# Greketrotny/RayZath

Hardware: AMD Instinct MI355X
Metric: Mrays/s (path segments, primary+secondary) at 1920x1080 depth 8 (higher is better)
Workload: dtype f32; 1 GPU; Cornell box 1920x1080 depth 8; max_depth=8, triangles=16, instances=8, traversal=workgroup-binned, integrator=CPU kernel (parity-checked), pipeline=resident (one kernel per step)

## Files before the change

### rayzath_amd/csrc/hiprz_device.hpp

```cpp
#pragma once
#include <hip/hip_runtime.h>
#include <stdint.h>

#include "hiprz.h"
#include "hiprz_end.hpp"
#include "hiprz_lds.hpp"
#include "hiprz_shard.hpp"

#define RZ_DEV __device__ __forceinline__
#include "hiprz_flat_pick.hpp"
#include "hiprz_pair_pick.hpp"

namespace hiprz {

#ifndef RZ_FUSED_SHARED_RCP
#define RZ_FUSED_SHARED_RCP 0
#endif
#ifndef RZ_TRACE_SHARED_RCP
#define RZ_TRACE_SHARED_RCP 1
#endif
#ifndef RZ_BATCH_SHARED_RCP
#define RZ_BATCH_SHARED_RCP 1
#endif
#ifndef RZ_FLAT_PACKED_BOXES
// ... 65 lines not shown
    uint32_t world_advance;
    uint32_t walk_h;
    uint32_t off_pairs;
    const float4* nodes64;
    uint32_t shadow_variant;
    const float4* shadow_nodes64;
    const uint32_t* shadow_order;
    uint32_t shadow_root;
    uint32_t sort_variant;
};

RZ_DEV void repoint_hot(DScene& v, const unsigned char* base) {
    v.nodes = reinterpret_cast<const float4*>(base + v.off_nodes);
    v.tlas_order = reinterpret_cast<const uint32_t*>(base + v.off_tlas_order);
    v.instances = reinterpret_cast<const float4*>(base + v.off_instances);
    v.tris = reinterpret_cast<const float4*>(base + v.off_tris);
    v.tri_attrs = reinterpret_cast<const float4*>(base + v.off_tri_attrs);
    v.materials = reinterpret_cast<const float4*>(base + v.off_materials);
    v.inst_materials = reinterpret_cast<const int32_t*>(base + v.off_inst_materials);
}

static_assert(sizeof(DScene) == 256, "off_pairs fills a padding word: the kernels' argument layout is what it was");
RZ_DEV const unsigned char* pair_section(const DScene& s) { return reinterpret_cast<const unsigned char*>(s.nodes) - s.off_nodes + s.off_pairs; }

struct DCamera {
    float position[3];
    float x_axis[3], y_axis[3], z_axis[3];
    uint32_t width, height;
    float tan_half_fov, aspect_ratio;
    float near_, far_;
    float focal_distance, aperture, exposure_time;
};

struct DConfig {
    uint32_t max_depth, spot_samples, direct_samples, seed;
    uint32_t flags;
};

struct DFrame {
    float4* st0;
    float4* st1;
    float2* st2;
    float4* accum;
    float4* hit0;
    uint32_t* hit1;
    float* depth;
// ... 1944 lines not shown
RZ_DEV col4 fetch_rgba8(const DScene& s, int32_t tex, float u, float v, Counters& cnt) {
    return from_u8(*reinterpret_cast<const uint32_t*>(s.texels + texel_offset<COUNT>(s, tex, u, v, 4u, cnt)));
}
template <bool COUNT>
RZ_DEV float fetch_r8(const DScene& s, int32_t tex, float u, float v, Counters& cnt) {
    return float(s.texels[texel_offset<COUNT>(s, tex, u, v, 1u, cnt)]) / 255.0f;
}
template <bool COUNT>
RZ_DEV float fetch_r32f(const DScene& s, int32_t tex, float u, float v, Counters& cnt) {
    return *reinterpret_cast<const float*>(s.texels + texel_offset<COUNT>(s, tex, u, v, 4u, cnt));
}

struct Surface {
    uint32_t surface_material, behind_material;
    float u, v;
    v3 normal, mapped_normal;
    col4 color;
    float metalness, roughness, emission;
    float fresnel, reflectance, tint_factor;
    float refr_x, refr_y;
    float surface_scattering;
};

template <bool COUNT, bool TEX = true>
RZ_DEV void analyze_intersection(const DScene& s, const Hit& hit, Surface& sf, Material& m, Counters& cnt, bool compat_filtering = false) {
    const uint32_t inst = uint32_t(hit.instance);
    const float4 i1 = s.instances[7 * inst + 1], i2 = s.instances[7 * inst + 2],
                 i3 = s.instances[7 * inst + 3], i4 = s.instances[7 * inst + 4];
    const v3 scale = xyz(i1), xa = xyz(i2), ya = xyz(i3), za = xyz(i4);
    const uint32_t material_base = __float_as_uint(i1.w), material_count = __float_as_uint(i2.w);

    const float4 ta = s.tris[3 * hit.triangle];
    const uint32_t flags = __float_as_uint(ta.w);
    const float4* at = s.tri_attrs + 6 * size_t(hit.triangle);

    uint32_t slot = flags & HIPRZ_TRI_MATERIAL_MASK;
    if (slot > 63u) slot = 63u;
    int32_t mat = -1;
    if (slot < material_count) mat = s.inst_materials[material_base + slot];
    sf.surface_material = mat < 0 ? HIPRZ_MATERIAL_DEFAULT : uint32_t(mat);
    sf.behind_material = hit.external ? sf.surface_material : HIPRZ_MATERIAL_WORLD;
    m = load_material(s, sf.surface_material);

    const bool has_texcrds = (flags & HIPRZ_TRI_HAS_TEXCRDS) != 0;
    float4 uv12 = make_float4(0, 0, 0, 0), uv3 = make_float4(0, 0, 0, 0);
    if (has_texcrds) {
        uv12 = at[4], uv3 = at[5];
        const float b3 = 1.0f - hit.bx - hit.by;
// ... 437 lines not shown
```

### rayzath_amd/csrc/hiprz_end.hpp

```cpp
#pragma once
#define RZ_END 0xFFFFFFFFu
#define RZ_PAIR_RECORD_BYTES 72u
```

### rayzath_amd/csrc/hiprz_kernels.hpp

```cpp
#pragma once
#include <hip/hip_runtime.h>

#include "hiprz.h"
#include "hiprz_device.hpp"
#include "hiprz_compat.hpp"

namespace hiprz {

struct PathState {
    Ray ray;
    col4 color;
    uint32_t material, depth;
};

template <bool LDS_SCENE>
RZ_DEV uint32_t stage_scene(DScene& s, unsigned char* lds) {
    if constexpr (LDS_SCENE) {
        float4* dst = reinterpret_cast<float4*>(lds);
        const uint32_t n16 = s.hot_bytes >> 4;
        for (uint32_t i = threadIdx.x; i < n16; i += 256u) dst[i] = s.hot[i];
        __syncthreads();
        repoint_hot(s, lds);
        return s.hot_bytes;
    }
// ... 61 lines not shown
        return closest_hit_flat<COUNT, RCP>(s, world, workspace, active, ray, hit, cnt);
    } else if constexpr (MODE == 2) {
        return closest_hit_binned<COUNT, RCP>(s, workspace, active, ray, hit, cnt);
    } else {
        hit.instance = -1, hit.triangle = 0, hit.bx = hit.by = 0.0f, hit.external = true;
        return active ? closest_hit<MODE, COUNT, RCP>(s, lds_column, ray, hit, cnt) : 0;
    }
}

template <bool COUNT, bool TEX, bool COMPAT>
RZ_DEV void fetch_color_emission(const DScene& s, const Material& m, uint32_t flags, bool filtering, Surface& sf, Counters& cnt) {
    if (COMPAT && (flags & HIPRZ_COMPAT_TEXTURE_MULT)) {
        sf.color = compat_opacity_color<COUNT>(s, m, sf.u, sf.v, true, filtering, cnt);
        sf.emission = m.emission;
        if (m.emission_map >= 0) sf.emission *= filtering ? compat_fetch<COUNT>(s, m.emission_map, sf.u, sf.v, cnt).r : fetch_r32f<COUNT>(s, m.emission_map, sf.u, sf.v, cnt);
    } else {
        sf.color = from_u8(m.color);
        if (TEX && m.texture >= 0) sf.color = filtering ? compat_fetch<COUNT>(s, m.texture, sf.u, sf.v, cnt) : fetch_rgba8<COUNT>(s, m.texture, sf.u, sf.v, cnt);
        sf.color.a = 1.0f - sf.color.a;
        sf.emission = TEX && m.emission_map >= 0 ? (filtering ? compat_fetch<COUNT>(s, m.emission_map, sf.u, sf.v, cnt).r : fetch_r32f<COUNT>(s, m.emission_map, sf.u, sf.v, cnt)) : m.emission;
    }
}

template <bool COUNT, int SHADOW = 1>
RZ_DEV void shade_segment(const DScene& s, const DCamera& cam, const DConfig& cfg, const PixelId& p, PathState& ps, uint32_t pass,
                          int found, const Hit& hit, const ShadowCtx& lds_column, Counters& cnt, col4& final_color, bool& path_continues,
                          Rng* shared_rng = nullptr) {
    constexpr bool COMPAT = shadow_mode_compat(SHADOW);
    Ray& ray = ps.ray;
    col4& ray_color = ps.color;
    uint32_t& ray_material = ps.material;
    uint32_t& depth = ps.depth;
    const uint32_t pixel_idx = p.y * cam.width + p.x;
    Rng own_rng(float(p.x) / float(cam.width), float(p.y) / float(cam.height), seed_value(cfg.seed, pass, (pixel_idx + depth) & 255u));
    Rng& rng = COMPAT ? *shared_rng : own_rng;
    const bool filtering = COMPAT && (cfg.flags & HIPRZ_COMPAT_FILTERING) != 0u;

    final_color = splat(0.0f);
    Surface sf;
    sf.surface_material = sf.behind_material = HIPRZ_MATERIAL_WORLD;
    sf.u = sf.v = 0.0f;
    sf.normal = sf.mapped_normal = V3(0.0f, 0.0f, 0.0f);
    sf.fresnel = 1.0f, sf.reflectance = 0.0f, sf.tint_factor = 0.0f, sf.refr_x = sf.refr_y = 0.0f;
    sf.metalness = sf.roughness = 0.0f;

    constexpr bool TEX = SHADOW != RZ_SHADOW_PLAIN;
    Material m;
    if (found == 2) {
        analyze_intersection<COUNT, TEX>(s, hit, sf, m, cnt, filtering);
    } else if (COMPAT && found == 3) {
        m = load_material(s, ray_material);
        sf.surface_material = sf.behind_material = ray_material;
        sf.normal = sf.mapped_normal = ray.d;
        if (TEX) {
            sf.u = -(0.5f + (RZ_ATAN2F(ray.d.z, ray.d.x) / (RZ_PI_F * 2.0f)));
            sf.v = 0.5f + (RZ_ASINF(ray.d.y) / RZ_PI_F);
        }
    } else {
        m = load_material(s, HIPRZ_MATERIAL_WORLD);
        if (TEX && (found == 1 || (COMPAT && found == 0))) {
            sf.u = -(0.5f + (RZ_ATAN2F(ray.d.z, ray.d.x) / (RZ_PI_F * 2.0f)));
            sf.v = 0.5f + (RZ_ASINF(ray.d.y) / RZ_PI_F);
        }
    }
    sf.surface_scattering = m.scattering;
    fetch_color_emission<COUNT, TEX, COMPAT>(s, m, cfg.flags, filtering, sf, cnt);
    if (COMPAT && (cfg.flags & HIPRZ_COMPAT_BEER_LAMBERT)) {
        col4 medium = from_u8(load_material(s, ray_material).color);
        medium.a = 1.0f - medium.a;
        ray_color = ray_color * (medium * RZ_POWF(medium.a, ray.far_));
    }
    if (sf.emission > 0.0f) final_color = final_color + (ray_color * sf.color) * sf.emission;
// ... 17 lines not shown
        if constexpr (shadow_mode_defers(SHADOW)) {
            lds_column.defer_done = true;
            lds_column.defer_a = ray_color, lds_column.defer_b = lerp(splat(1.0f), sf.color, sf.metalness);
        } else if constexpr (SHADOW == RZ_SHADOW_NONE || SHADOW == RZ_SHADOW_PLAIN) {
            (void)direct;
        } else {
            final_color = final_color + (direct * ray_color) * lerp(splat(1.0f), sf.color, sf.metalness);
        }
        ray_color = lerp(ray_color, ray_color * sf.color, sf.tint_factor);
    }
    path_continues = depth < cfg.max_depth;
    if (path_continues) {
        ray.o = point;
        ray.d = next_direction;
    } else {
        RZ_COUNT(finished);
        generate_antialiased_ray(cam, ray, p.x, p.y, rng);
        ray_material = HIPRZ_MATERIAL_WORLD;
        ray_color = splat(1.0f);
        depth = 0u;
    }
}

template <bool FIRST, bool COUNT, int SHADOW = 1>
RZ_DEV void shade_and_store(const DScene& s, const DCamera& cam, const DConfig& cfg, const DFrame& f, const PixelId& p, PathState& ps,
                            int found, const Hit& hit, const ShadowCtx& lds_column, Counters& cnt, Rng* shared_rng = nullptr) {
    const float hit_distance = ps.ray.far_;
    col4 final_color;
    bool path_continues;
    shade_segment<COUNT, SHADOW>(s, cam, cfg, p, ps, FIRST ? 0u : *f.pass, found, hit, lds_column, cnt, final_color, path_continues, shared_rng);
    const Ray& ray = ps.ray;
    const col4& ray_color = ps.color;
    const uint32_t ray_material = ps.material, depth = ps.depth;

    if constexpr (FIRST) f.depth[p.local] = hit_distance;
    if constexpr (shadow_mode_defers(SHADOW)) {
        const uint32_t bits = (path_continues ? 1u : 0u) | (lds_column.defer_done ? 2u : 0u) | (lds_column.defer_mask << 2);
        float4* rec = f.nee + size_t(p.local) * f.nee_quads;
        rec[0] = make_float4(final_color.r, final_color.g, final_color.b, __uint_as_float(bits));
        if (lds_column.defer_done) {
            rec[2] = make_float4(lds_column.defer_a.r, lds_column.defer_a.g, lds_column.defer_a.b, lds_column.defer_a.a);
            rec[3] = make_float4(lds_column.defer_b.r, lds_column.defer_b.g, lds_column.defer_b.b, lds_column.defer_b.a);
        }
    } else {
        col4 value;
        if constexpr (FIRST) {
            value = col4{final_color.r, final_color.g, final_color.b, float(!path_continues)};
        } else {
            const float4 acc = f.accum[p.local];
            value = col4{acc.x + final_color.r, acc.y + final_color.g, acc.z + final_color.b, acc.w + float(!path_continues)};
        }
        f.accum[p.local] = make_float4(value.r, value.g, value.b, value.a);
    }
// ... 47 lines not shown
    DScene s = scene_in;
    unsigned char* workspace = rz_lds + stage_scene<LDS_SCENE>(s, rz_lds);
    uint32_t* lds_column = stack_column<MODE>(workspace);
    const PixelId p = pixel_of_thread(f, cam, blockIdx.x, threadIdx.x);
    Counters cnt;
    PathState ps;
    load_path<FIRST>(f, cam, p, ps);
    Hit hit;
    int found;
    const auto world = walk_world<MODE>(s);
    if constexpr (binned_mode(MODE)) {
        static_assert(kFusedParkBytes == 4u * 256u * sizeof(uint32_t), "park [4][256]");
        uint32_t* park = reinterpret_cast<uint32_t*>(workspace + BinnedLds::kFixedBytes + (s.world_stack_entries + s.mesh_stack_entries) * 1024u);
        park[0 * 256 + threadIdx.x] = __float_as_uint(ps.color.r), park[1 * 256 + threadIdx.x] = __float_as_uint(ps.color.g);
        park[2 * 256 + threadIdx.x] = __float_as_uint(ps.color.b), park[3 * 256 + threadIdx.x] = ps.material | (ps.depth << 16);
        found = trace_path<MODE, COUNT, RZ_FUSED_SHARED_RCP != 0>(s, world, workspace, lds_column, p.active, ps.ray, hit, cnt);
        ps.color = col4{__uint_as_float(park[0 * 256 + threadIdx.x]), __uint_as_float(park[1 * 256 + threadIdx.x]),
                        __uint_as_float(park[2 * 256 + threadIdx.x]), 1.0f};
        const uint32_t bits = park[3 * 256 + threadIdx.x];
        ps.material = bits & 0xFFFFu, ps.depth = bits >> 16;
    } else {
        found = trace_path<MODE, COUNT, RZ_FUSED_SHARED_RCP != 0>(s, world, workspace, lds_column, p.active, ps.ray, hit, cnt);
    }
    if (p.active) shade_and_store<FIRST, COUNT>(s, cam, cfg, f, p, ps, found, hit, ShadowCtx{lds_column, TopCache{nullptr, nullptr, 0u}}, cnt);
    flush_counters<COUNT>(f, p.active ? 1u : 0u, cnt);
}

template <bool COUNT, int MODE, int SHADING, bool SC1 = false>
RZ_DEV void batch_tile(const DScene& s, const DCamera& cam, const DConfig& cfg, const DFrame& f, unsigned char* workspace, uint32_t* park,
                       const PixelId& p, uint32_t pass0, uint32_t n_passes, bool tonemap_out, Counters& cnt) {
    uint32_t* lds_column = stack_column<MODE>(workspace);
    PathState ps;
    load_path<false, SC1>(f, cam, p, ps);
    {
        const float4 acc = p.active ? load_state<SC1>(f.accum + p.local) : make_float4(0.0f, 0.0f, 0.0f, 0.0f);
        park[4 * 256] = __float_as_uint(acc.x), park[5 * 256] = __float_as_uint(acc.y);
        park[6 * 256] = __float_as_uint(acc.z), park[7 * 256] = __float_as_uint(acc.w);
    }
    const auto world = walk_world<MODE>(s);
    for (uint32_t i = 0; i < n_passes; ++i) {
        if (i != 0u && p.active) {
            ps.ray.d = normalized(ps.ray.d);
            ps.ray.near_ = 0.0f, ps.ray.far_ = RZ_FLT_MAX;
            if (ps.depth == 0u) ps.ray.near_ = cam.near_, ps.ray.far_ = cam.far_;
        }
        Hit hit;
        int found;
        if constexpr (binned_mode(MODE)) {
            park[0 * 256] = __float_as_uint(ps.color.r), park[1 * 256] = __float_as_uint(ps.color.g);
            park[2 * 256] = __float_as_uint(ps.color.b), park[3 * 256] = ps.material | (ps.depth << 16);
            found = trace_path<MODE, COUNT, RZ_BATCH_SHARED_RCP != 0>(s, world, workspace, lds_column, p.active, ps.ray, hit, cnt);
            ps.color = col4{__uint_as_float(park[0 * 256]), __uint_as_float(park[1 * 256]), __uint_as_float(park[2 * 256]), 1.0f};
            const uint32_t bits = park[3 * 256];
            ps.material = bits & 0xFFFFu, ps.depth = bits >> 16;
        } else {
            found = trace_path<MODE, COUNT, RZ_BATCH_SHARED_RCP != 0>(s, world, workspace, lds_column, p.active, ps.ray, hit, cnt);
        }
        if (p.active) {
            col4 final_color;
            bool path_continues;
            shade_segment<COUNT, SHADING>(s, cam, cfg, p, ps, pass0 + i, found, hit, ShadowCtx{lds_column, TopCache{nullptr, nullptr, 0u}}, cnt, final_color, path_continues);
            park[4 * 256] = __float_as_uint(__uint_as_float(park[4 * 256]) + final_color.r);
            park[5 * 256] = __float_as_uint(__uint_as_float(park[5 * 256]) + final_color.g);
            park[6 * 256] = __float_as_uint(__uint_as_float(park[6 * 256]) + final_color.b);
            park[7 * 256] = __float_as_uint(__uint_as_float(park[7 * 256]) + float(!path_continues));
        }
    }
    if (p.active) {
        const float4 acc = make_float4(__uint_as_float(park[4 * 256]), __uint_as_float(park[5 * 256]), __uint_as_float(park[6 * 256]),
                                       __uint_as_float(park[7 * 256]));
        store_state<SC1>(f.accum + p.local, acc);
        store_state<SC1>(f.st0 + p.local, make_float4(ps.ray.o.x, ps.ray.o.y, ps.ray.o.z, ps.ray.d.x));
        store_state<SC1>(f.st1 + p.local, make_float4(ps.ray.d.y, ps.ray.d.z, ps.color.r, ps.color.g));
        store_state<SC1>(f.st2 + p.local, make_float2(ps.color.b, __uint_as_float((ps.material & 0xFFFFu) | (ps.depth << 16))));
        if (tonemap_out) f.rgba8[p.local] = tonemap(col4{acc.x, acc.y, acc.z, acc.w}, cam.aperture, cam.exposure_time);
    }
}

template <bool COUNT, int MODE, bool LDS_SCENE, int SHADING, int WAVES = RZ_MIN_WAVES>
__global__ void __launch_bounds__(256, WAVES) rz_batch_kernel(const DScene scene_in, const DCamera cam, const DConfig cfg, const DFrame f,
                                                                      uint32_t n_passes, uint32_t park_offset) {
    extern __shared__ __attribute__((aligned(16))) unsigned char rz_lds[];
    const unsigned long long t_start = __builtin_readcyclecounter();
    const uint32_t unit = (f.launch_order && !f.xcd_swizzle) ? f.launch_order[blockIdx.x] : blockIdx.x;
    const PixelId p = pixel_of_thread(f, cam, unit, threadIdx.x);
    if (!p.tile_inside) return;
    DScene s = scene_in;
    unsigned char* workspace = rz_lds + stage_scene<LDS_SCENE>(s, rz_lds);
    Counters cnt;
    uint32_t* park = reinterpret_cast<uint32_t*>(workspace + park_offset) + threadIdx.x;
    batch_tile<COUNT, MODE, SHADING>(s, cam, cfg, f, workspace, park, p, *f.pass, n_passes, true, cnt);
    if (f.unit_cost && threadIdx.x == 0u) {
        const unsigned long long dt = (__builtin_readcyclecounter() - t_start) >> 4;
        f.unit_cost[unit] = dt < 0x00FFFFFFull ? uint32_t(dt) : 0x00FFFFFFu;
    }
    flush_counters<COUNT>(f, p.active ? n_passes : 0u, cnt);
}

template <bool COUNT, int MODE, bool LDS_SCENE, int SHADING, int WAVES = RZ_MIN_WAVES>
__global__ void __launch_bounds__(256, WAVES) rz_batch_seg_kernel(const DScene scene_in, const DCamera cam, const DConfig cfg, const DFrame f,
                                                                          uint32_t n_passes, uint32_t park_offset, uint32_t segments, uint32_t n_units,
                                                                          uint32_t* seg) {
    extern __shared__ __attribute__((aligned(16))) unsigned char rz_lds[];
    DScene s = scene_in;
    unsigned char* workspace = rz_lds + stage_scene<LDS_SCENE>(s, rz_lds);
    uint32_t* park = reinterpret_cast<uint32_t*>(workspace + park_offset) + threadIdx.x;
    uint32_t* item_slot = reinterpret_cast<uint32_t*>(workspace + park_offset + 8u * 1024u);
    const uint32_t n_items = segments * n_units, pass_base = *f.pass;
    uint32_t base = 0u;
    if (threadIdx.x == 0u) base = __hip_atomic_load(&seg[2], __ATOMIC_RELAXED, __HIP_MEMORY_SCOPE_AGENT);
    for (;;) {
        if (threadIdx.x == 0u) item_slot[0] = __hip_atomic_fetch_add(&seg[0], 1u, __ATOMIC_RELAXED, __HIP_MEMORY_SCOPE_AGENT);
        __syncthreads();
        const uint32_t item = item_slot[0];
        if (item >= n_items) break;
        const uint32_t k = item / n_units, j = item - k * n_units;
        const uint32_t unit = (f.launch_order && !f.xcd_swizzle) ? f.launch_order[j] : j;
        const PixelId p = pixel_of_thread(f, cam, unit, threadIdx.x);
        if (p.tile_inside) {
            if (k != 0u) {
                if (threadIdx.x == 0u) {
                    for (uint32_t guard = 0u; __hip_atomic_load(&seg[kSegFlags + unit], __ATOMIC_RELAXED, __HIP_MEMORY_SCOPE_AGENT) != base + k;) {
                        __builtin_amdgcn_s_sleep(2);
                        if (++guard > kSegWaitLimit) break;
                    }
                    __builtin_amdgcn_fence(__ATOMIC_ACQUIRE, "wavefront");
                }
                __syncthreads();
            }
            const unsigned long long t_start = __builtin_readcyclecounter();
            const uint32_t first = k * n_passes / segments, end = (k + 1u) * n_passes / segments;
            Counters cnt;
            batch_tile<COUNT, MODE, SHADING, true>(s, cam, cfg, f, workspace, park, p, pass_base + first, end - first, k + 1u == segments, cnt);
            if (f.unit_cost && threadIdx.x == 0u) {
                const uint32_t before = k != 0u ? __hip_atomic_load(&f.unit_cost[unit], __ATOMIC_RELAXED, __HIP_MEMORY_SCOPE_AGENT) : 0u;
                const unsigned long long dt = ((__builtin_readcyclecounter() - t_start) >> 4) + before;
                __hip_atomic_store(&f.unit_cost[unit], dt < 0x00FFFFFFull ? uint32_t(dt) : 0x00FFFFFFu, __ATOMIC_RELAXED, __HIP_MEMORY_SCOPE_AGENT);
            }
            flush_counters<COUNT>(f, p.active ? end - first : 0u, cnt);
            if (k + 1u != segments) {
                asm volatile("s_waitcnt vmcnt(0)" ::: "memory");
                __syncthreads();
                if (threadIdx.x == 0u) __hip_atomic_store(&seg[kSegFlags + unit], base + k + 1u, __ATOMIC_RELAXED, __HIP_MEMORY_SCOPE_AGENT);
            }
        }
        __syncthreads();
    }
    if (threadIdx.x == 0u && __hip_atomic_fetch_add(&seg[1], 1u, __ATOMIC_ACQ_REL, __HIP_MEMORY_SCOPE_AGENT) == gridDim.x - 1u) {
        __hip_atomic_store(&seg[0], 0u, __ATOMIC_RELAXED, __HIP_MEMORY_SCOPE_AGENT);
        __hip_atomic_store(&seg[1], 0u, __ATOMIC_RELAXED, __HIP_MEMORY_SCOPE_AGENT);
        __hip_atomic_store(&seg[2], base + segments, __ATOMIC_RELAXED, __HIP_MEMORY_SCOPE_AGENT);
    }
}

template <bool COUNT, int SHADING, int MINW, bool ONE_LEAF_WORLD = false>
__global__ void __launch_bounds__(64, MINW) rz_wave_batch_kernel(const DScene s, const DCamera cam, const DConfig cfg, const DFrame f, uint32_t n_passes) {
// ... 161 lines not shown
        for (uint32_t i = threadIdx.x; i < top_n; i += 256u) ls[i] = s.node_skip[i];
        __syncthreads();
        shadow.lds_column = nullptr;
        shadow.top = TopCache{ln, ls, top_n};
    }
    const PixelId p = pixel_of_thread(f, cam, blockIdx.x, threadIdx.x);
    Counters cnt;
    if (p.active) {
        PathState ps;
        load_path<FIRST>(f, cam, p, ps);
        const float4 h0 = f.hit0[p.local];
        const uint32_t h1 = f.hit1[p.local];
        Hit hit;
        const int found = int((h1 >> 29) & 3u);
        ps.ray.far_ = h0.x;
        hit.bx = h0.y, hit.by = h0.z, hit.triangle = __float_as_uint(h0.w);
        hit.instance = found == 2 ? int32_t(h1 & 0x1FFFFFFFu) : -1;
        hit.external = (h1 & 0x80000000u) != 0u;
        shadow.nee = f.nee + size_t(p.local) * f.nee_quads;
        if constexpr (shadow_mode_compat(SHADOW)) {
            const uint32_t pass = FIRST ? 0u : *f.pass, pixel_idx = p.y * cam.width + p.x;
            Rng rng(float(p.x) / float(cam.width), float(p.y) / float(cam.height), seed_value(cfg.seed, pass, (pixel_idx + ps.depth) & 255u));
            if ((cfg.flags & HIPRZ_COMPAT_SCATTERING) && material_scattering(s, ps.material) > 1.0e-4f) (void)rng.unsignedUniform();
            shade_and_store<FIRST, COUNT, SHADOW>(s, cam, cfg, f, p, ps, found, hit, shadow, cnt, &rng);
        } else {
            shade_and_store<FIRST, COUNT, SHADOW>(s, cam, cfg, f, p, ps, found, hit, shadow, cnt);
        }
    } else if (f.sort_key && p.local < f.n_local_tiles * 256u) {
        f.sort_key[p.local] = 0x00FFFFFFu;
        if (f.shadow_key) f.shadow_key[p.local] = 0x00FFFFFFu;
    }
    flush_counters<COUNT>(f, p.active ? 1u : 0u, cnt);
}

template <bool FIRST, bool COUNT, int MINW>
__global__ void __launch_bounds__(64, MINW) rz_shadow_kernel(const DScene s, const DCamera cam, const DConfig cfg, const DFrame f, uint32_t top_n) {
    extern __shared__ __attribute__((aligned(16))) unsigned char rz_lds[];
    float4* ln = reinterpret_cast<float4*>(rz_lds);
    uint32_t* ls = reinterpret_cast<uint32_t*>(rz_lds + top_n * 32u);
    for (uint32_t i = threadIdx.x; i < 2u * top_n; i += 64u) ln[i] = s.nodes[i];
    for (uint32_t i = threadIdx.x; i < top_n; i += 64u) ls[i] = s.node_skip[i];
    const uint32_t slot = blockIdx.x * 64u + threadIdx.x;
    const uint32_t* order = f.shadow_perm ? f.shadow_perm : f.perm;
    const PixelId p = pixel_of_local(f, cam, order ? order[slot] : slot);
    Counters cnt;
    if (p.active) {
        const ShadowCtx sc{nullptr, TopCache{ln, ls, top_n}};
        const float4* rec = f.nee + size_t(p.local) * f.nee_quads;
        const float4 base = rec[0];
// ... 182 lines not shown
```

### rayzath_amd/csrc/hiprz_scene.hip

```cpp
#include <hip/hip_runtime.h>

#include <algorithm>
#include <cstdio>
#include <cstdlib>
#include <cstring>
#include <string>
#include <vector>

#include "hiprz.h"
#include "hiprz_ctx.hpp"
#include "hiprz_device.hpp"
#include "hiprz_scene_host.hpp"

using namespace hiprz;

#define RZ_FANOUT_OTHER_DEVICES(c, call)                                                                                       \
    for (hiprz_ctx* p : (c)->peers) {                                                                                         \
        if (p->device == (c)->device) continue;                                                                               \
        const int rz_rc = (call);                                                                                             \
        if (rz_rc != HIPRZ_OK) return fail(c, rz_rc, "device " + std::to_string(p->device) + ": " + p->error);              \
    }

namespace {

// ... 46 lines not shown
uint32_t env_u32(const char* name, uint32_t otherwise) {
    const char* v = std::getenv(name);
    return v ? uint32_t(std::atoi(v)) : otherwise;
}
uint32_t sort_variant_for(const hiprz_ctx* c, uint32_t n_lights) { return n_lights && c->shadow_sort == 0 ? 0u : 4u; }

int build_shadow_world_tree(hiprz_ctx* c, const std::vector<hiprz_instance>& dinst, DScene& d) {
    d.shadow_nodes64 = nullptr, d.shadow_order = nullptr, d.shadow_root = RZ_END;
    const std::vector<uint32_t>& members = c->world_members;
    if (!c->shadow_tree || members.empty() || members.size() > 160u) return HIPRZ_OK;
    std::vector<uint32_t> rec, order;
    build_shadow_tree(dinst, members, rec, order);
    (void)hipSetDevice(c->device);
    RZ_HIP(c, c->shadow_nodes64.resize(rec.size()));
    RZ_HIP(c, c->shadow_order.resize(order.size()));
    RZ_HIP(c, hipStreamSynchronize(c->stream));
    RZ_HIP(c, hipMemcpy(c->shadow_nodes64.ptr, rec.data(), rec.size() * sizeof(uint32_t), hipMemcpyHostToDevice));
    RZ_HIP(c, hipMemcpy(c->shadow_order.ptr, order.data(), order.size() * sizeof(uint32_t), hipMemcpyHostToDevice));
    d.shadow_nodes64 = reinterpret_cast<const float4*>(c->shadow_nodes64.ptr), d.shadow_order = c->shadow_order.ptr, d.shadow_root = 0u;
    return HIPRZ_OK;
}


int copy_scene(hiprz_ctx* c, const hiprz_scene& sc, const PackedScene& packed, bool device_trees) {
    (void)hipSetDevice(c->device);
    if (packed.pair_section.empty()) {
        RZ_HIP(c, c->hot.assign(packed.blob.data(), packed.blob.size(), c->stream));
    } else {
        std::vector<uint8_t> hot(packed.blob);
        hot.insert(hot.end(), packed.pair_section.begin(), packed.pair_section.end());
        RZ_HIP(c, c->hot.assign(hot.data(), hot.size(), c->stream));
        RZ_HIP(c, hipStreamSynchronize(c->stream));
    }
    RZ_HIP(c, c->node_skip.assign(packed.skip.data(), packed.skip.size(), c->stream));
    if (device_trees) {
        hiprz_node unused{};
        unused.meta = HIPRZ_NODE_LEAF;
        std::vector<hiprz_node> all(packed.node_capacity, unused);
        std::copy(packed.nodes.begin(), packed.nodes.end(), all.begin());
        RZ_HIP(c, c->dev_nodes.assign(reinterpret_cast<const uint8_t*>(all.data()), all.size() * sizeof(hiprz_node), c->stream));
        RZ_HIP(c, hipStreamSynchronize(c->stream));
    }
    RZ_HIP(c, c->nodes64.assign(packed.nodes64.data(), packed.nodes64.size(), c->stream));
    RZ_HIP(c, c->textures.assign(sc.textures, sc.n_textures, c->stream));
    RZ_HIP(c, c->texels.assign(sc.texels, sc.texel_bytes, c->stream));
    RZ_HIP(c, c->spot_lights.assign(sc.spot_lights, sc.n_spot_lights, c->stream));
    RZ_HIP(c, c->direct_lights.assign(sc.direct_lights, sc.n_direct_lights, c->stream));
    RZ_HIP(c, hipStreamSynchronize(c->stream));
    return HIPRZ_OK;
}

void bind_tunables(hiprz_ctx* c, DScene& d, uint32_t n_lights) {
    d.walk_k = env_u32("HIPRZ_WALK_K", 4u), d.walk_l = env_u32("HIPRZ_WALK_L", 8u);
// ... 82 lines not shown
        rc = derive_tables(scene, chk, derived);
    }
    if (message && len) std::snprintf(message, len, "%s", chk.error.c_str());
    return rc;
}

int hiprz_upload_scene(hiprz_ctx* c, const hiprz_scene* sc) {
    if (!c) return HIPRZ_ERR_INVALID;
    RZ_FANOUT_OTHER_DEVICES(c, hiprz_upload_scene(p, sc));
    SceneChange change(c, SceneChange::kInvalidateGraphs | SceneChange::kResolvePeerPipelines);
    StageTimer timer;
    std::string error;
    SceneCheck chk;
    if (check_scene(sc, chk) != HIPRZ_OK) return fail(c, HIPRZ_ERR_INVALID, "upload_scene: " + chk.error);
    c->build_sah = c->device_sah || c->tree_mode == HIPRZ_TREE_AUTO;
    ChosenTrees trees;
    if (choose_trees(sc, c->tree_mode, kLdsSceneLimit, chk, trees, error) != HIPRZ_OK) return fail(c, HIPRZ_ERR_INVALID, error);
    if (trees.own_trees) c->timings.set("rebuild mesh trees", timer.ms());
    DerivedTables derived;
    if (derive_tables(&trees.scene, chk, derived) != HIPRZ_OK) return fail(c, HIPRZ_ERR_INVALID, "upload_scene: " + chk.error);
    c->have_scene = false;
    PackedScene packed;
    if (pack_scene(trees, std::move(derived), packed, error) != HIPRZ_OK) return scene_lost(c, fail(c, HIPRZ_ERR_INVALID, error));
    int rc = copy_scene(c, trees.scene, packed, trees.device_trees());
    if (rc != HIPRZ_OK) return scene_lost(c, rc);
    bind_scene(c, trees, packed, chk);
    if (trees.device_trees()) rc = build_device_trees(c, packed);
    if (rc != HIPRZ_OK) return scene_lost(c, rc);
    rc = build_shadow_world_tree(c, packed.instances, c->dscene);
    if (rc != HIPRZ_OK) return scene_lost(c, rc);
    c->have_scene = true;
    resolve_pipeline(c);
    c->timings.set("upload scene", timer.ms());
    return restart_after_geometry_change(c);
}

int hiprz_update_shading(hiprz_ctx* c, const hiprz_material* materials, uint32_t n_materials, const hiprz_spot_light* spot_lights,
                         uint32_t n_spot_lights, const hiprz_direct_light* direct_lights, uint32_t n_direct_lights) {
    if (!c) return HIPRZ_ERR_INVALID;
    RZ_FANOUT_OTHER_DEVICES(c, hiprz_update_shading(p, materials, n_materials, spot_lights, n_spot_lights, direct_lights, n_direct_lights));
    SceneChange change(c, SceneChange::kInPlace);
    if (!c->have_scene) return fail(c, HIPRZ_ERR_STATE, "update_shading before upload_scene");
    const uint32_t uploaded = (c->dscene.off_inst_materials - c->dscene.off_materials) / uint32_t(sizeof(hiprz_material));
    if (!materials || n_materials < 2u || ((n_materials * sizeof(hiprz_material) + 15u) & ~size_t(15)) != size_t(c->dscene.off_inst_materials - c->dscene.off_materials))
        return fail(c, HIPRZ_ERR_INVALID, "update_shading: the scene was uploaded with " + std::to_string(uploaded) + " material slots");
    if ((n_spot_lights && !spot_lights) || (n_direct_lights && !direct_lights)) return fail(c, HIPRZ_ERR_INVALID, "update_shading: null array with non-zero count");
    std::vector<hiprz_texture> tex(c->n_textures);
// ... 116 lines not shown
```

### rayzath_amd/csrc/hiprz_scene_host.cpp

```cpp
#include "hiprz_scene_host.hpp"

#include <algorithm>

namespace hiprz {

namespace {
struct TreeCheck {
    const hiprz_scene* sc;
    std::vector<uint32_t>& skip;
    std::vector<uint8_t> visited;
    uint32_t max_depth = 0;
    std::string error;
    std::vector<uint32_t> world_leaves;

    bool walk(uint32_t root, bool is_world) {
        struct Item {
            uint32_t node, skip, depth;
        };
        std::vector<Item> stack{{root, RZ_END, 1u}};
        while (!stack.empty()) {
            const Item it = stack.back();
            stack.pop_back();
            if (it.node >= sc->n_nodes) return err("node index out of range");
            if (visited[it.node]) return err("node reachable twice (trees must be disjoint and acyclic)");
            visited[it.node] = 1;
// ... 355 lines not shown
                }
            }
            table[i] = uint16_t(first_of_root[root]), any = true;
        }
        if (any && table_bytes + records.size() <= kPairSectionLimit) {
            out.pair_section.assign((table_bytes + records.size() + 15u) & ~size_t(15), 0);
            std::memcpy(out.pair_section.data(), table.data(), table_bytes);
            if (!records.empty()) std::memcpy(out.pair_section.data() + table_bytes, records.data(), records.size());
        }
        if (out.hot_bytes() > 0xFFFFFFF0ull) {
            error = "scene geometry exceeds 4 GiB";
            return HIPRZ_ERR_INVALID;
        }
    }
    std::vector<uint8_t> member(sc->n_instances ? sc->n_instances : 1u, 0);
    for (uint32_t k = 0; k < sc->n_tlas_order; ++k)
        if (sc->tlas_order[k] < sc->n_instances) member[sc->tlas_order[k]] = 1;
    out.world_members.clear();
    for (uint32_t i = 0; i < sc->n_instances; ++i)
        if (member[i]) out.world_members.push_back(i);
    return HIPRZ_OK;
}

uint32_t enter_device_roots(std::vector<hiprz_instance>& instances, const std::vector<uint32_t>& instance_mesh, const std::vector<DeviceMesh>& meshes,
                            uint32_t world_slots) {
    for (size_t i = 0; i < instances.size(); ++i)
        if (instance_mesh[i] != RZ_END && meshes[instance_mesh[i]].region != RZ_END) instances[i].blas_root = meshes[instance_mesh[i]].region;
    uint32_t emitted = world_slots;
    for (const auto& m : meshes) emitted += m.n_slots;
    return emitted;
}

void build_shadow_tree(const std::vector<hiprz_instance>& dinst, const std::vector<uint32_t>& members, std::vector<uint32_t>& rec,
                       std::vector<uint32_t>& order) {
    auto box_of = [&](uint32_t i) { return packed_instance_box(dinst[i]); };
    auto grow = [](InstanceBox& b, const InstanceBox& o) {
        for (int a = 0; a < 3; ++a) b.mn[a] = std::min(b.mn[a], o.mn[a]), b.mx[a] = std::max(b.mx[a], o.mx[a]);
    };
    auto area = [](const InstanceBox& b) {
        const float x = b.mx[0] - b.mn[0], y = b.mx[1] - b.mn[1], z = b.mx[2] - b.mn[2];
        return x * y + y * z + z * x;
    };
    const uint32_t n = uint32_t(members.size());
    order = members, rec.assign(size_t(2u * n) * 16u, RZ_END);
    std::vector<uint32_t> sorted, best;
    std::vector<float> left_area;
// ... 50 lines not shown
```

### rayzath_amd/csrc/hiprz_scene_host.hpp

```cpp
#pragma once
#include <cstdint>
#include <cstring>
#include <string>
#include <vector>

#include "hiprz.h"
#include "hiprz_end.hpp"

namespace hiprz {

constexpr uint32_t kLeafMax = 4u;
constexpr uint32_t kPairRecordBytes = RZ_PAIR_RECORD_BYTES;
constexpr uint16_t kPairNone = 0xFFFFu;
constexpr size_t kPairSectionLimit = 8u * 0xFFFEu;

struct DeviceMesh {
    uint32_t tri_first = 0, n_tris = 0;
    uint32_t ref_first = 0;
    uint32_t region = 0xFFFFFFFFu;
    uint32_t leaf_slot = 0xFFFFFFFFu;
    uint32_t n_slots = 0;
    float bb_min[3] = {0, 0, 0}, bb_max[3] = {0, 0, 0};
};
uint32_t device_build_regions(std::vector<DeviceMesh>& meshes, uint32_t first_free_slot);
// ... 66 lines not shown
int choose_trees(const hiprz_scene* sc, uint32_t tree_mode, size_t lds_limit, SceneCheck& chk, ChosenTrees& out, std::string& error);

struct PackedScene {
    std::vector<uint8_t> blob;
    uint32_t off_nodes = 0, off_tlas_order = 0, off_instances = 0, off_tris = 0, off_tri_attrs = 0, off_materials = 0, off_inst_materials = 0;
    std::vector<uint32_t> new_index;
    std::vector<hiprz_node> nodes;
    std::vector<uint32_t> skip;
    std::vector<uint32_t> nodes64;
    std::vector<hiprz_instance> instances;
    std::vector<uint32_t> world_members;
    bool fast_div = true;
    float bounds_min[3] = {0, 0, 0}, bounds_scale[3] = {0, 0, 0};
    uint32_t tlas_root = 0;
    bool flat_world = false;
    std::vector<uint8_t> pair_section;
    size_t hot_bytes() const { return blob.size() + pair_section.size(); }
    std::vector<DeviceMesh> device_meshes;
    std::vector<uint32_t> instance_mesh;
    uint32_t world_region = 0, node_capacity = 0;
};
int pack_scene(const ChosenTrees& trees, DerivedTables&& derived, PackedScene& out, std::string& error, bool pair_records = true);

uint32_t enter_device_roots(std::vector<hiprz_instance>& instances, const std::vector<uint32_t>& instance_mesh, const std::vector<DeviceMesh>& meshes,
                            uint32_t world_slots);

void build_shadow_tree(const std::vector<hiprz_instance>& instances, const std::vector<uint32_t>& members, std::vector<uint32_t>& records,
                       std::vector<uint32_t>& order);

}
```

Baseline: 12430 Mrays/s.

## Precompute per-instance-triangle surface normal records in the hot scene section

```diff
diff --git a/rayzath_amd/csrc/hiprz_device.hpp b/rayzath_amd/csrc/hiprz_device.hpp
--- a/rayzath_amd/csrc/hiprz_device.hpp
+++ b/rayzath_amd/csrc/hiprz_device.hpp
@@ -111,6 +111,11 @@
 
 static_assert(sizeof(DScene) == 256, "off_pairs fills a padding word: the kernels' argument layout is what it was");
 RZ_DEV const unsigned char* pair_section(const DScene& s) { return reinterpret_cast<const unsigned char*>(s.nodes) - s.off_nodes + s.off_pairs; }
+
+#ifndef RZ_SURFACE_RECORDS
+#define RZ_SURFACE_RECORDS 1
+#endif
+RZ_DEV const float4* surface_section(const DScene& s) { return s.hot + ((s.hot_bytes + 15u) >> 4); }
 
 struct DCamera {
     float position[3];
@@ -2101,8 +2106,47 @@
     float surface_scattering;
 };
 
-template <bool COUNT, bool TEX = true>
+template <bool TEX>
+RZ_DEV bool surface_from_record(const DScene& s, const Hit& hit, Surface& sf, Material& m) {
+    const float4* section = surface_section(s);
+    const uint32_t pair = reinterpret_cast<const uint32_t*>(section)[uint32_t(hit.instance)] + hit.triangle;
+    const float4* rec = section + ((s.n_instances + 3u) >> 2) + (size_t(pair) * 4u + (hit.external ? 2u : 0u));
+    const float4 ra = rec[0], rb = rec[1];
+    const uint32_t valid = __float_as_uint(rb.w);
+    if (!(valid & RZ_SURFACE_NORMAL_VALID)) return false;
+    sf.surface_material = __float_as_uint(ra.w);
+    sf.behind_material = hit.external ? sf.surface_material : HIPRZ_MATERIAL_WORLD;
+    m = load_material(s, sf.surface_material);
+    if (TEX && m.normal_map >= 0) return false;
+    sf.normal = xyz(ra);
+    if (TEX || !(valid & RZ_SURFACE_MAPPED_VALID)) {
+        const uint32_t flags = __float_as_uint(s.tris[3 * hit.triangle].w);
+        const float4* at = s.tri_attrs + 6 * size_t(hit.triangle);
+        if (TEX && (flags & HIPRZ_TRI_HAS_TEXCRDS)) {
+            const float4 uv12 = at[4], uv3 = at[5];
+            const float b3 = 1.0f - hit.bx - hit.by;
+            sf.u = uv12.x * b3 + uv12.z * hit.bx + uv3.x * hit.by;
+            sf.v = uv12.y * b3 + uv12.w * hit.bx + uv3.y * hit.by;
+        }
+        if (!(valid & RZ_SURFACE_MAPPED_VALID)) {
+            const uint32_t inst = uint32_t(hit.instance);
+            const v3 scale = xyz(s.instances[7 * inst + 1]), xa = xyz(s.instances[7 * inst + 2]), ya = xyz(s.instances[7 * inst + 3]),
+                     za = xyz(s.instances[7 * inst + 4]);
+            v3 mn = xyz(at[3]);
+            if (flags & HIPRZ_TRI_HAS_NORMALS) mn = normalized(xyz(at[0]) * (1.0f - hit.bx - hit.by) + xyz(at[1]) * hit.bx + xyz(at[2]) * hit.by);
+            sf.mapped_normal = normalized(transform_forward(xa, ya, za, mn / scale)) * (float(hit.external) * 2.0f - 1.0f);
+            return true;
+        }
+    }
+    sf.mapped_normal = xyz(rb);
+    return true;
+}
+
+template <bool COUNT, bool TEX = true, bool RECORDS = false>
 RZ_DEV void analyze_intersection(const DScene& s, const Hit& hit, Surface& sf, Material& m, Counters& cnt, bool compat_filtering = false) {
+    if constexpr (RECORDS) {
+        if (surface_from_record<TEX>(s, hit, sf, m)) return;
+    }
     const uint32_t inst = uint32_t(hit.instance);
     const float4 i1 = s.instances[7 * inst + 1], i2 = s.instances[7 * inst + 2],
                  i3 = s.instances[7 * inst + 3], i4 = s.instances[7 * inst + 4];
diff --git a/rayzath_amd/csrc/hiprz_end.hpp b/rayzath_amd/csrc/hiprz_end.hpp
--- a/rayzath_amd/csrc/hiprz_end.hpp
+++ b/rayzath_amd/csrc/hiprz_end.hpp
@@ -1,3 +1,6 @@
 #pragma once
 #define RZ_END 0xFFFFFFFFu
 #define RZ_PAIR_RECORD_BYTES 72u
+#define RZ_SURFACE_RECORD_BYTES 32u
+#define RZ_SURFACE_NORMAL_VALID 1u
+#define RZ_SURFACE_MAPPED_VALID 2u
diff --git a/rayzath_amd/csrc/hiprz_kernels.hpp b/rayzath_amd/csrc/hiprz_kernels.hpp
--- a/rayzath_amd/csrc/hiprz_kernels.hpp
+++ b/rayzath_amd/csrc/hiprz_kernels.hpp
@@ -107,7 +107,8 @@
     }
 }
 
-template <bool COUNT, int SHADOW = 1>
+constexpr bool surface_records(bool lds_scene) { return lds_scene && RZ_SURFACE_RECORDS != 0; }
+template <bool COUNT, int SHADOW = 1, bool RECORDS = false>
 RZ_DEV void shade_segment(const DScene& s, const DCamera& cam, const DConfig& cfg, const PixelId& p, PathState& ps, uint32_t pass,
                           int found, const Hit& hit, const ShadowCtx& lds_column, Counters& cnt, col4& final_color, bool& path_continues,
                           Rng* shared_rng = nullptr) {
@@ -132,7 +133,7 @@
     constexpr bool TEX = SHADOW != RZ_SHADOW_PLAIN;
     Material m;
     if (found == 2) {
-        analyze_intersection<COUNT, TEX>(s, hit, sf, m, cnt, filtering);
+        analyze_intersection<COUNT, TEX, RECORDS>(s, hit, sf, m, cnt, filtering);
     } else if (COMPAT && found == 3) {
         m = load_material(s, ray_material);
         sf.surface_material = sf.behind_material = ray_material;
@@ -196,13 +197,13 @@
     }
 }
 
-template <bool FIRST, bool COUNT, int SHADOW = 1>
+template <bool FIRST, bool COUNT, int SHADOW = 1, bool RECORDS = false>
 RZ_DEV void shade_and_store(const DScene& s, const DCamera& cam, const DConfig& cfg, const DFrame& f, const PixelId& p, PathState& ps,
                             int found, const Hit& hit, const ShadowCtx& lds_column, Counters& cnt, Rng* shared_rng = nullptr) {
     const float hit_distance = ps.ray.far_;
     col4 final_color;
     bool path_continues;
-    shade_segment<COUNT, SHADOW>(s, cam, cfg, p, ps, FIRST ? 0u : *f.pass, found, hit, lds_column, cnt, final_color, path_continues, shared_rng);
+    shade_segment<COUNT, SHADOW, RECORDS>(s, cam, cfg, p, ps, FIRST ? 0u : *f.pass, found, hit, lds_column, cnt, final_color, path_continues, shared_rng);
     const Ray& ray = ps.ray;
     const col4& ray_color = ps.color;
     const uint32_t ray_material = ps.material, depth = ps.depth;
@@ -296,11 +297,11 @@
     } else {
         found = trace_path<MODE, COUNT, RZ_FUSED_SHARED_RCP != 0>(s, world, workspace, lds_column, p.active, ps.ray, hit, cnt);
     }
-    if (p.active) shade_and_store<FIRST, COUNT>(s, cam, cfg, f, p, ps, found, hit, ShadowCtx{lds_column, TopCache{nullptr, nullptr, 0u}}, cnt);
+    if (p.active) shade_and_store<FIRST, COUNT, 1, surface_records(LDS_SCENE)>(s, cam, cfg, f, p, ps, found, hit, ShadowCtx{lds_column, TopCache{nullptr, nullptr, 0u}}, cnt);
     flush_counters<COUNT>(f, p.active ? 1u : 0u, cnt);
 }
 
-template <bool COUNT, int MODE, int SHADING, bool SC1 = false>
+template <bool COUNT, int MODE, int SHADING, bool SC1 = false, bool RECORDS = false>
 RZ_DEV void batch_tile(const DScene& s, const DCamera& cam, const DConfig& cfg, const DFrame& f, unsigned char* workspace, uint32_t* park,
                        const PixelId& p, uint32_t pass0, uint32_t n_passes, bool tonemap_out, Counters& cnt) {
     uint32_t* lds_column = stack_column<MODE>(workspace);
@@ -333,7 +334,7 @@
         if (p.active) {
             col4 final_color;
             bool path_continues;
-            shade_segment<COUNT, SHADING>(s, cam, cfg, p, ps, pass0 + i, found, hit, ShadowCtx{lds_column, TopCache{nullptr, nullptr, 0u}}, cnt, final_color, path_continues);
+            shade_segment<COUNT, SHADING, RECORDS>(s, cam, cfg, p, ps, pass0 + i, found, hit, ShadowCtx{lds_column, TopCache{nullptr, nullptr, 0u}}, cnt, final_color, path_continues);
             park[4 * 256] = __float_as_uint(__uint_as_float(park[4 * 256]) + final_color.r);
             park[5 * 256] = __float_as_uint(__uint_as_float(park[5 * 256]) + final_color.g);
             park[6 * 256] = __float_as_uint(__uint_as_float(park[6 * 256]) + final_color.b);
@@ -363,7 +364,7 @@
     unsigned char* workspace = rz_lds + stage_scene<LDS_SCENE>(s, rz_lds);
     Counters cnt;
     uint32_t* park = reinterpret_cast<uint32_t*>(workspace + park_offset) + threadIdx.x;
-    batch_tile<COUNT, MODE, SHADING>(s, cam, cfg, f, workspace, park, p, *f.pass, n_passes, true, cnt);
+    batch_tile<COUNT, MODE, SHADING, false, surface_records(LDS_SCENE)>(s, cam, cfg, f, workspace, park, p, *f.pass, n_passes, true, cnt);
     if (f.unit_cost && threadIdx.x == 0u) {
         const unsigned long long dt = (__builtin_readcyclecounter() - t_start) >> 4;
         f.unit_cost[unit] = dt < 0x00FFFFFFull ? uint32_t(dt) : 0x00FFFFFFu;
@@ -405,7 +406,7 @@
             const unsigned long long t_start = __builtin_readcyclecounter();
             const uint32_t first = k * n_passes / segments, end = (k + 1u) * n_passes / segments;
             Counters cnt;
-            batch_tile<COUNT, MODE, SHADING, true>(s, cam, cfg, f, workspace, park, p, pass_base + first, end - first, k + 1u == segments, cnt);
+            batch_tile<COUNT, MODE, SHADING, true, surface_records(LDS_SCENE)>(s, cam, cfg, f, workspace, park, p, pass_base + first, end - first, k + 1u == segments, cnt);
             if (f.unit_cost && threadIdx.x == 0u) {
                 const uint32_t before = k != 0u ? __hip_atomic_load(&f.unit_cost[unit], __ATOMIC_RELAXED, __HIP_MEMORY_SCOPE_AGENT) : 0u;
                 const unsigned long long dt = ((__builtin_readcyclecounter() - t_start) >> 4) + before;
@@ -613,9 +614,9 @@
             const uint32_t pass = FIRST ? 0u : *f.pass, pixel_idx = p.y * cam.width + p.x;
             Rng rng(float(p.x) / float(cam.width), float(p.y) / float(cam.height), seed_value(cfg.seed, pass, (pixel_idx + ps.depth) & 255u));
             if ((cfg.flags & HIPRZ_COMPAT_SCATTERING) && material_scattering(s, ps.material) > 1.0e-4f) (void)rng.unsignedUniform();
-            shade_and_store<FIRST, COUNT, SHADOW>(s, cam, cfg, f, p, ps, found, hit, shadow, cnt, &rng);
+            shade_and_store<FIRST, COUNT, SHADOW, surface_records(LDS_SCENE)>(s, cam, cfg, f, p, ps, found, hit, shadow, cnt, &rng);
         } else {
-            shade_and_store<FIRST, COUNT, SHADOW>(s, cam, cfg, f, p, ps, found, hit, shadow, cnt);
+            shade_and_store<FIRST, COUNT, SHADOW, surface_records(LDS_SCENE)>(s, cam, cfg, f, p, ps, found, hit, shadow, cnt);
         }
     } else if (f.sort_key && p.local < f.n_local_tiles * 256u) {
         f.sort_key[p.local] = 0x00FFFFFFu;
diff --git a/rayzath_amd/csrc/hiprz_scene.hip b/rayzath_amd/csrc/hiprz_scene.hip
--- a/rayzath_amd/csrc/hiprz_scene.hip
+++ b/rayzath_amd/csrc/hiprz_scene.hip
@@ -92,13 +92,15 @@
 }
 
 
-int copy_scene(hiprz_ctx* c, const hiprz_scene& sc, const PackedScene& packed, bool device_trees) {
-    (void)hipSetDevice(c->device);
-    if (packed.pair_section.empty()) {
+int copy_scene(hiprz_ctx* c, const hiprz_scene& sc, const PackedScene& packed, const std::vector<uint8_t>& surface_section, bool device_trees) {
+    (void)hipSetDevice(c->device);
+    if (packed.pair_section.empty() && surface_section.empty()) {
         RZ_HIP(c, c->hot.assign(packed.blob.data(), packed.blob.size(), c->stream));
     } else {
         std::vector<uint8_t> hot(packed.blob);
         hot.insert(hot.end(), packed.pair_section.begin(), packed.pair_section.end());
+        hot.resize((hot.size() + 15u) & ~size_t(15), 0);
+        hot.insert(hot.end(), surface_section.begin(), surface_section.end());
         RZ_HIP(c, c->hot.assign(hot.data(), hot.size(), c->stream));
         RZ_HIP(c, hipStreamSynchronize(c->stream));
     }
@@ -227,7 +229,8 @@
     c->have_scene = false;
     PackedScene packed;
     if (pack_scene(trees, std::move(derived), packed, error) != HIPRZ_OK) return scene_lost(c, fail(c, HIPRZ_ERR_INVALID, error));
-    int rc = copy_scene(c, trees.scene, packed, trees.device_trees());
+    const std::vector<uint8_t> surface_section = pack_surface_section(trees, packed, chk.world_depth + chk.mesh_depth + 2u, kLdsPerCu);
+    int rc = copy_scene(c, trees.scene, packed, surface_section, trees.device_trees());
     if (rc != HIPRZ_OK) return scene_lost(c, rc);
     bind_scene(c, trees, packed, chk);
     if (trees.device_trees()) rc = build_device_trees(c, packed);
diff --git a/rayzath_amd/csrc/hiprz_scene_host.cpp b/rayzath_amd/csrc/hiprz_scene_host.cpp
--- a/rayzath_amd/csrc/hiprz_scene_host.cpp
+++ b/rayzath_amd/csrc/hiprz_scene_host.cpp
@@ -1,6 +1,7 @@
 #include "hiprz_scene_host.hpp"
 
 #include <algorithm>
+#include <cmath>
 
 namespace hiprz {
 
@@ -402,6 +403,112 @@
     return HIPRZ_OK;
 }
 
+namespace {
+
+struct SurfaceMath {
+    bool bad = false;
+    float see(float x) {
+        uint32_t b;
+        std::memcpy(&b, &x, 4);
+        const uint32_t e = (b >> 23) & 0xFFu;
+        if (e == 0xFFu || (e == 0u && (b & 0x007FFFFFu) != 0u)) bad = true;
+        return x;
+    }
+    void scaled(const float v[3], float s, float out[3]) {
+        for (int a = 0; a < 3; ++a) out[a] = see(v[a] * s);
+    }
+    void divided(const float v[3], const float d[3], float out[3]) {
+        for (int a = 0; a < 3; ++a) out[a] = see(v[a] / d[a]);
+    }
+    void forward(const hiprz_instance& in, const float v[3], float out[3]) {
+        for (int a = 0; a < 3; ++a) {
+            const float x = see(in.x_axis[a] * v[0]), y = see(in.y_axis[a] * v[1]), z = see(in.z_axis[a] * v[2]);
+            out[a] = see(see(x + y) + z);
+        }
+    }
+    void normalize(const float v[3], float out[3]) {
+        const float xx = see(v[0] * v[0]), yy = see(v[1] * v[1]), zz = see(v[2] * v[2]);
+        const float r = see(1.0f / see(std::sqrt(see(see(xx + yy) + zz))));
+        scaled(v, r, out);
+    }
+};
+
+}
+
+std::vector<uint8_t> pack_surface_section(const ChosenTrees& trees, const PackedScene& packed, uint32_t stack_entries, size_t lds_limit) {
+    std::vector<uint8_t> section;
+    const hiprz_scene* sc = &trees.scene;
+    if (trees.own_trees || sc->n_instances == 0u || packed.hot_bytes() + size_t(stack_entries) * 1024u > lds_limit) return section;
+    struct Range {
+        uint32_t lo = RZ_END, hi = 0u;
+    };
+    std::vector<Range> range_of_root(sc->n_nodes);
+    std::vector<uint8_t> ranged(sc->n_nodes, 0);
+    const uint32_t table_words = (sc->n_instances + 3u) & ~3u;
+    std::vector<uint32_t> table(table_words, 0u);
+    std::vector<uint32_t> words;
+    std::vector<uint32_t> todo;
+    for (const uint32_t i : packed.world_members) {
+        const hiprz_instance& in = sc->instances[i];
+        const uint32_t root = in.blas_root;
+        if (!ranged[root]) {
+            Range r;
+            todo.assign(1, root);
+            while (!todo.empty()) {
+                const hiprz_node& n = sc->nodes[todo.back()];
+                todo.pop_back();
+                if (n.meta & HIPRZ_NODE_LEAF) {
+                    const uint32_t count = n.meta & HIPRZ_NODE_COUNT_MASK;
+                    if (count) r.lo = std::min(r.lo, n.begin), r.hi = std::max(r.hi, n.begin + count);
+                } else {
+                    todo.push_back(n.begin), todo.push_back(n.begin + 1u);
+                }
+            }
+            range_of_root[root] = r, ranged[root] = 1;
+        }
+        const Range r = range_of_root[root];
+        if (r.lo >= r.hi) continue;
+        table[i] = uint32_t(words.size() / 16u) - r.lo;
+        float scale_in[3];
+        SurfaceMath placement;
+        for (int a = 0; a < 3; ++a) scale_in[a] = placement.see(in.scale[a]), placement.see(in.x_axis[a]), placement.see(in.y_axis[a]), placement.see(in.z_axis[a]);
+        for (uint32_t t = r.lo; t < r.hi; ++t) {
+            const uint32_t flags = sc->tris[t].material_flags;
+            uint32_t slot = flags & HIPRZ_TRI_MATERIAL_MASK;
+            if (slot > 63u) slot = 63u;
+            int32_t mat = -1;
+            if (slot < in.material_count && uint64_t(in.material_base) + slot < sc->n_inst_materials) mat = sc->inst_materials[in.material_base + slot];
+            const uint32_t surface_material = mat < 0 ? HIPRZ_MATERIAL_DEFAULT : uint32_t(mat);
+            const float* face_normal = sc->tri_attrs[t].face_normal;
+            for (uint32_t external = 0; external < 2u; ++external) {
+                const float ef = float(external) * 2.0f - 1.0f;
+                SurfaceMath math = placement;
+                for (int a = 0; a < 3; ++a) math.see(face_normal[a]);
+                float v[3], w[3], normal[3], mapped[3];
+                math.scaled(face_normal, ef, v);
+                math.divided(v, scale_in, w);
+                math.forward(in, w, v);
+                math.normalize(v, normal);
+                math.divided(face_normal, scale_in, w);
+                math.forward(in, w, v);
+                math.normalize(v, w);
+                math.scaled(w, ef, mapped);
+                uint32_t valid = 0u;
+                if (!math.bad) valid = kSurfaceNormalValid | ((flags & HIPRZ_TRI_HAS_NORMALS) ? 0u : kSurfaceMappedValid);
+                uint32_t rec[8];
+                std::memcpy(rec, normal, 12), std::memcpy(rec + 4, mapped, 12);
+                rec[3] = surface_material, rec[7] = valid;
+                words.insert(words.end(), rec, rec + 8);
+            }
+        }
+    }
+    static_assert(kSurfaceRecordBytes == 32u, "two float4 per record");
+    section.resize(4u * (size_t(table_words) + words.size()));
+    std::memcpy(section.data(), table.data(), 4u * size_t(table_words));
+    if (!words.empty()) std::memcpy(section.data() + 4u * size_t(table_words), words.data(), 4u * words.size());
+    return section;
+}
+
 uint32_t enter_device_roots(std::vector<hiprz_instance>& instances, const std::vector<uint32_t>& instance_mesh, const std::vector<DeviceMesh>& meshes,
                             uint32_t world_slots) {
     for (size_t i = 0; i < instances.size(); ++i)
diff --git a/rayzath_amd/csrc/hiprz_scene_host.hpp b/rayzath_amd/csrc/hiprz_scene_host.hpp
--- a/rayzath_amd/csrc/hiprz_scene_host.hpp
+++ b/rayzath_amd/csrc/hiprz_scene_host.hpp
@@ -112,6 +112,10 @@
 };
 int pack_scene(const ChosenTrees& trees, DerivedTables&& derived, PackedScene& out, std::string& error, bool pair_records = true);
 
+constexpr uint32_t kSurfaceRecordBytes = RZ_SURFACE_RECORD_BYTES;
+constexpr uint32_t kSurfaceNormalValid = RZ_SURFACE_NORMAL_VALID, kSurfaceMappedValid = RZ_SURFACE_MAPPED_VALID;
+std::vector<uint8_t> pack_surface_section(const ChosenTrees& trees, const PackedScene& packed, uint32_t stack_entries, size_t lds_limit);
+
 uint32_t enter_device_roots(std::vector<hiprz_instance>& instances, const std::vector<uint32_t>& instance_mesh, const std::vector<DeviceMesh>& meshes,
                             uint32_t world_slots);
 
```

Result: faster. 12850 Mrays/s (median of 6 runs) (+3.4%).
